# ChrisDud0257/SSL

Measured on AMD Instinct MI355X. Metric: SSG-loss edge-pixels/sec (fwd+bwd) 3x256x256 k_s=25 k_w=9, higher is better.
Workload: dtype f32; 1 GPU; C2: batch 16 x 3x256x256 per GPU, Laplacian mask, k_s=25 k_w=9 sigma=1.0, L1+KL w=1e3, SSGs materialised; launch=per-kernel, ranks_seen=1, edge_px_rank0=76466, images_rank0=16, input_checksum=c1391ff6908574f6, gradient_accumulation=fixed-point integer atomics (bit-reproducible, the shipped default), prewarm_steps=1949, parallelism=images sharded x1, no data-path collective

## Files before the change

include/ssg_hip.h:

```cpp
#ifndef SSG_HIP_H
#define SSG_HIP_H

#include <stddef.h>
#include <stdint.h>

#ifdef __cplusplus
extern "C" {
#endif

typedef void *ssg_stream_t;

#define SSG_E_BADARG (-1)
#define SSG_E_TOOLARGE (-2)
#define SSG_E_WORKSPACE (-3)
#define SSG_E_IMAGESMALL (-4)
#define SSG_E_ALIGN (-5)
#define SSG_E_PLAN (-6)

int ssg_abi_version(void);
const char *ssg_status_string(int status);
int ssg_device_status(ssg_stream_t stream);

int ssg_set_operator_plan_threshold(int positions);
int ssg_operator_pool_trim(void);
int ssg_compute_similarity(const float *image, const int *pos, float *out,
                           int mc, int psize, int ksize, int height, int width,
                           int channel, ssg_stream_t stream);

int ssg_compute_similarity_backward(const float *image, const float *grads,
                                    const int *pos, float *image_grads, int mc,
                                    int psize, int ksize, int height, int width,
                                    int channel, ssg_stream_t stream);

size_t ssg_edge_scratch_bytes(int B, int H, int W);
size_t ssg_forward_plan_bytes(int B, int H, int W, int capacity);
int ssg_set_dense_threshold(int edge_pixels_per_tile);
int ssg_set_overlap(int mode);
int ssg_last_overlap_assignment(void);
int ssg_set_tiny_step(int on);
int ssg_edge_list(const void *mask, int mask_kind, int mask_channels, int B,
                  int H, int W, int mask_stride, float lap_threshold,
                  int plan_ks ,
                  int *edges, int capacity, int *counts,
                  int *rank_map , int *tile_order ,
                  int *fwd_plan , void *scratch,
                  ssg_stream_t stream);

int ssg_edge_mask_laplacian(const float *gt, int B, int H, int W,
                            float lap_threshold, int mask_stride,
                            uint8_t *mask_out, ssg_stream_t stream);

int ssg_map_forward(const float *img, const float *img2, int B, int C, int H,
                    int W, const int *edges, const int *tile_order ,
                    const int *rank_map ,
                    const int *fwd_plan ,
                    const int *n_edges_dev, int n_rows,
                    int ks, int kw, float sigma, float eps, int generalization,
                    float *ssg, float *ssg2,
                    double *row_scale ,
                    ssg_stream_t stream);

size_t ssg_backward_scratch_bytes(int n_rows, int ks);
int ssg_map_backward(const float *img, int B, int C, int H, int W,
                     const int *edges, const int *tile_order ,
                     const int *rank_map ,
                     const int *fwd_plan ,
                     const int *n_edges_dev, int n_rows,
                     int ks, int kw, float sigma, int generalization,
                     const float *ssg, const float *grad_ssg, float *grad_img,
                     void *scratch , void *grad_fix ,
                     ssg_stream_t stream);

size_t ssg_grad_fix_bytes(int B, int C, int H, int W);

size_t ssg_loss_scratch_bytes(int B, int H, int W, int n_rows, int ks);
int ssg_loss_backward(const float *sr, int B, int C, int H, int W,
                      const int *edges, const int *tile_order ,
                      const int *rank_map ,
                      const int *fwd_plan ,
                      const int *n_edges_dev, int n_rows,
                      int ks, int kw, float sigma, int generalization,
                      float *ssg_sr, float *ssg_gt, float w_l1,
                      float w_kl, const float *upstream ,
                      float *loss_out, float *grad_sr ,
                      void *scratch, void *grad_fix ,
                      const double *row_scale , int rows_are_scratch, ssg_stream_t stream);

size_t ssg_criteria_scratch_bytes(void);
int ssg_criteria_sums(const float *pred, const float *target, size_t n, void *scratch, float *sums_out,
                      ssg_stream_t stream);
int ssg_criteria_grad(const float *pred, const float *target, size_t n, const float *coef, float *grad_pred,
                      ssg_stream_t stream);

size_t ssg_loss_workspace_bytes(int B, int H, int W, int capacity, int ks);
size_t ssg_loss_rows_bytes(int capacity, int ks);
size_t ssg_loss_tm_bytes(int capacity, int ks);
int ssg_loss_workspace_layout(int B, int H, int W, int capacity, int ks, int fused, size_t out[9]);
int ssg_loss_fwd_bwd(const float *sr, const float *gt, const void *mask,
                     int mask_kind, int mask_channels, int B, int C, int H,
                     int W, int ks, int kw, float sigma, float eps,
                     int generalization, float w_l1, float w_kl, int mask_stride,
                     float lap_threshold, int capacity, float *ssg_sr ,
                     float *ssg_gt, int *counts, float *loss_out, float *grad_sr,
                     void *workspace, size_t workspace_bytes,
                     void *grad_fix , ssg_stream_t stream);

int ssg_loss_step(const float *sr, const float *gt, const void *mask,
                  int mask_kind, int mask_channels, int B, int C, int H,
                  int W, int ks, int kw, float sigma, float eps,
                  int generalization, float w_l1, float w_kl, int mask_stride,
                  float lap_threshold, int capacity, float *ssg_sr ,
                  float *ssg_gt, int *counts, float *loss_out, float *grad_sr,
                  void *workspace, size_t workspace_bytes,
                  void *grad_fix , ssg_stream_t stream);

int ssg_augment_crop(const void *src, void *dst, int elem_bytes, int B, int C, int Hs, int Ws, int Ho, int Wo,
                     const int *params, ssg_stream_t stream);
int ssg_pool_swap(void *queue, void *batch, size_t sample_bytes, const int *slots, int b, ssg_stream_t stream);

int ssg_filter2d(const float *img, const float *kernels, float *out, int B, int C, int H, int W, int k, int n_kernels,
                 ssg_stream_t stream);
int ssg_diffjpeg(const float *img, float *out, int B, int H, int W, const float *quality_dev, float quality,
                 ssg_stream_t stream);
size_t ssg_usm_scratch_bytes(int B, int C, int H, int W);
int ssg_usm_sharp(const float *img, float *out, int B, int C, int H, int W, int radius, float sigma, float weight,
                  float threshold, void *scratch, size_t scratch_bytes, ssg_stream_t stream);

int ssg_resize(const float *img, float *out, int B, int C, int Hi, int Wi, int Ho, int Wo, int mode,
               double scale_factor_h, double scale_factor_w, ssg_stream_t stream);
int ssg_clamp_round(const float *img, float *out, size_t n, int clip, int rounds, ssg_stream_t stream);
int ssg_gaussian_noise(const float *img, float *out, const float *field_color, const float *field_gray,
                       const float *sigma, const float *gray, int B, int C, int H, int W, int clip, int rounds,
                       ssg_stream_t stream);
size_t ssg_poisson_scratch_bytes(int B);
int ssg_poisson_rates(const float *img, float *rate_color, float *rate_gray, float *vals, void *scratch, int B, int C,
                      int H, int W, ssg_stream_t stream);
int ssg_poisson_noise(const float *img, float *out, const float *draw_color, const float *draw_gray, const float *vals,
                      const float *scale, const float *gray, int B, int C, int H, int W, int clip, int rounds,
                      ssg_stream_t stream);

size_t ssg_ldl_workspace_bytes(int B, int H, int W);
int ssg_artifact_map(const float *output, const float *gt, const float *ema , int B, int C, int H, int W,
                     int k, float *w_out, void *workspace, size_t workspace_bytes, ssg_stream_t stream);
int ssg_artifact_map_backward(const float *output, const float *gt, const float *ema ,
                              const float *grad_w, int B, int C, int H, int W, int k, float *grad_output,
                              void *workspace, size_t workspace_bytes, ssg_stream_t stream);
int ssg_ldl_loss(const float *output, const float *gt, const float *ema , int B, int C, int H, int W,
                 int k, float loss_weight, int mean, float *loss_out, float *grad_output ,
                 void *workspace, size_t workspace_bytes, ssg_stream_t stream);
int ssg_local_variance(const float *residual, int B, int H, int W, int k, float *v_out ,
                       const float *grad_v , float *grad_residual , void *workspace,
                       size_t workspace_bytes, ssg_stream_t stream);

size_t ssg_bbl_workspace_bytes(int B, int C, int H, int W, int k, int stride);
int ssg_bbl_search(const float *x, const float *gt, int B, int C, int H, int W, int k, int stride, float alpha,
                   float beta, int *ind_out, float *p1_out , float *sel_out ,
                   void *workspace, size_t workspace_bytes, ssg_stream_t stream);
int ssg_bbl_loss(const float *x, const float *gt, int B, int C, int H, int W, int k, int stride, float alpha,
                 float beta, float loss_weight, int mean, float *loss_out, float *grad_x ,
                 int *ind_out , void *workspace, size_t workspace_bytes, ssg_stream_t stream);
int ssg_flat_mask(const float *img, int B, int H, int W, int k, float thresh, float *mask_out, ssg_stream_t stream);

#ifdef SSG_PROFILE
int ssg_set_profile_mask(int mask);
int ssg_prof_occupancy(int which);
int ssg_prof_strip_times(unsigned long long *host, int n);
int ssg_prof_set_lds_poison(int on, unsigned pattern);
#endif

const char *ssg_kernel_name(int ks, int kw, int backward);

#ifdef __cplusplus
}
#endif
#endif
```

ssl_amd/_lib.py:

```python
import ctypes
import os
import subprocess

_HERE = os.path.dirname(os.path.abspath(__file__))
CSRC = os.path.join(_HERE, "csrc")
SO_PATH = os.path.join(CSRC, "libssg_hip.so")
PROF_SO_PATH = os.path.join(CSRC, "libssg_hip_prof.so")
HEADER = os.path.join(os.path.dirname(_HERE), "include", "ssg_hip.h")

_vp, _i, _f, _sz = ctypes.c_void_p, ctypes.c_int, ctypes.c_float, ctypes.c_size_t

PROTOTYPES = {
    "ssg_abi_version": (_i, []),
    "ssg_status_string": (ctypes.c_char_p, [_i]),
    "ssg_compute_similarity": (_i, [_vp, _vp, _vp, _i, _i, _i, _i, _i, _i, _vp]),
    "ssg_compute_similarity_backward": (_i, [_vp, _vp, _vp, _vp, _i, _i, _i, _i, _i, _i, _vp]),
    "ssg_edge_scratch_bytes": (_sz, [_i, _i, _i]),
    "ssg_forward_plan_bytes": (_sz, [_i, _i, _i, _i]),
    "ssg_set_dense_threshold": (_i, [_i]),
    "ssg_set_overlap": (_i, [_i]),
    "ssg_last_overlap_assignment": (_i, []),
    "ssg_set_tiny_step": (_i, [_i]),
    "ssg_edge_list": (_i, [_vp, _i, _i, _i, _i, _i, _i, _f, _i, _vp, _i, _vp, _vp, _vp, _vp, _vp, _vp]),
    "ssg_edge_mask_laplacian": (_i, [_vp, _i, _i, _i, _f, _i, _vp, _vp]),
    "ssg_map_forward": (_i, [_vp, _vp, _i, _i, _i, _i, _vp, _vp, _vp, _vp, _vp, _i, _i, _i, _f, _f, _i, _vp, _vp,
                             _vp, _vp]),
    "ssg_backward_scratch_bytes": (_sz, [_i, _i]),
    "ssg_map_backward": (_i, [_vp, _i, _i, _i, _i, _vp, _vp, _vp, _vp, _vp, _i, _i, _i, _f, _i, _vp, _vp, _vp, _vp,
                              _vp, _vp]),
    "ssg_grad_fix_bytes": (_sz, [_i, _i, _i, _i]),
    "ssg_loss_scratch_bytes": (_sz, [_i, _i, _i, _i, _i]),
    "ssg_loss_backward": (_i, [_vp, _i, _i, _i, _i, _vp, _vp, _vp, _vp, _vp, _i, _i, _i, _f, _i, _vp, _vp, _f, _f,
                               _vp, _vp, _vp, _vp, _vp, _vp, _i, _vp]),
    "ssg_loss_workspace_bytes": (_sz, [_i, _i, _i, _i, _i]),
    "ssg_loss_rows_bytes": (_sz, [_i, _i]),
    "ssg_loss_tm_bytes": (_sz, [_i, _i]),
    "ssg_loss_workspace_layout": (_i, [_i, _i, _i, _i, _i, _i, ctypes.POINTER(ctypes.c_size_t)]),
    "ssg_filter2d": (_i, [_vp, _vp, _vp, _i, _i, _i, _i, _i, _i, _vp]),
    "ssg_diffjpeg": (_i, [_vp, _vp, _i, _i, _i, _vp, _f, _vp]),
    "ssg_usm_scratch_bytes": (_sz, [_i, _i, _i, _i]),
    "ssg_usm_sharp": (_i, [_vp, _vp, _i, _i, _i, _i, _i, _f, _f, _f, _vp, _sz, _vp]),
    "ssg_loss_fwd_bwd": (_i, [_vp, _vp, _vp, _i, _i, _i, _i, _i, _i, _i, _i, _f, _f, _i, _f, _f, _i, _f, _i, _vp, _vp,
                              _vp, _vp, _vp, _vp, _sz, _vp, _vp]),
    "ssg_loss_step": (_i, [_vp, _vp, _vp, _i, _i, _i, _i, _i, _i, _i, _i, _f, _f, _i, _f, _f, _i, _f, _i, _vp, _vp,
                           _vp, _vp, _vp, _vp, _sz, _vp, _vp]),
    "ssg_augment_crop": (_i, [_vp, _vp, _i, _i, _i, _i, _i, _i, _i, _vp, _vp]),
    "ssg_pool_swap": (_i, [_vp, _vp, _sz, _vp, _i, _vp]),
    "ssg_resize": (_i, [_vp, _vp, _i, _i, _i, _i, _i, _i, _i, ctypes.c_double, ctypes.c_double, _vp]),
    "ssg_clamp_round": (_i, [_vp, _vp, _sz, _i, _i, _vp]),
    "ssg_gaussian_noise": (_i, [_vp, _vp, _vp, _vp, _vp, _vp, _i, _i, _i, _i, _i, _i, _vp]),
    "ssg_poisson_scratch_bytes": (_sz, [_i]),
    "ssg_poisson_rates": (_i, [_vp, _vp, _vp, _vp, _vp, _i, _i, _i, _i, _vp]),
    "ssg_poisson_noise": (_i, [_vp, _vp, _vp, _vp, _vp, _vp, _vp, _i, _i, _i, _i, _i, _i, _vp]),
    "ssg_kernel_name": (ctypes.c_char_p, [_i, _i, _i]),
    "ssg_ldl_workspace_bytes": (_sz, [_i, _i, _i]),
    "ssg_artifact_map": (_i, [_vp, _vp, _vp, _i, _i, _i, _i, _i, _vp, _vp, _sz, _vp]),
    "ssg_artifact_map_backward": (_i, [_vp, _vp, _vp, _vp, _i, _i, _i, _i, _i, _vp, _vp, _sz, _vp]),
    "ssg_ldl_loss": (_i, [_vp, _vp, _vp, _i, _i, _i, _i, _i, _f, _i, _vp, _vp, _vp, _sz, _vp]),
    "ssg_local_variance": (_i, [_vp, _i, _i, _i, _i, _vp, _vp, _vp, _vp, _sz, _vp]),
    "ssg_bbl_workspace_bytes": (_sz, [_i, _i, _i, _i, _i, _i]),
    "ssg_bbl_search": (_i, [_vp, _vp, _i, _i, _i, _i, _i, _i, _f, _f, _vp, _vp, _vp, _vp, _sz, _vp]),
    "ssg_bbl_loss": (_i, [_vp, _vp, _i, _i, _i, _i, _i, _i, _f, _f, _f, _i, _vp, _vp, _vp, _vp, _sz, _vp]),
    "ssg_flat_mask": (_i, [_vp, _i, _i, _i, _i, _f, _vp, _vp]),
    "ssg_ref_compute_similarity": (None, [_vp, _vp, _vp, _i, _i, _i, _i, _i, _i]),
    "ssg_ref_compute_similarity_backward": (None, [_vp, _vp, _vp, _vp, _i, _i, _i, _i, _i, _i]),
    "ssg_last_status": (_i, []),
    "ssg_device_status": (_i, [_vp]),
    "ssg_set_operator_plan_threshold": (_i, [_i]),
    "ssg_operator_pool_trim": (_i, []),
    "ssg_criteria_scratch_bytes": (_sz, []),
    "ssg_criteria_sums": (_i, [_vp, _vp, _sz, _vp, _vp, _vp]),
    "ssg_criteria_grad": (_i, [_vp, _vp, _sz, _vp, _vp, _vp]),
}
PROF_PROTOTYPES = {"ssg_set_profile_mask": (_i, [_i]), "ssg_prof_occupancy": (_i, [_i]),
                   "ssg_prof_set_lds_poison": (_i, [_i, ctypes.c_uint])}
CXX_SYMBOLS = ("_Z19_compute_similarityPKfPKiPfiiiiii", "_Z28_compute_similarity_backwardPKfS0_PKiPfiiiiii")


def build(force=False, verbose=False):
    cmd = ["make", "-C", CSRC, "-j4"] + (["-B"] if force else [])
    out = subprocess.run(cmd, stdout=subprocess.PIPE, stderr=subprocess.STDOUT, text=True)
    if verbose or out.returncode:
        print(out.stdout)
    if out.returncode:
        raise RuntimeError("building libssg_hip.so failed (see output above)")
    return SO_PATH


_lib = None
_prof = None


def _load(path, prototypes):
    import torch
    if torch.cuda.is_available():
        torch.cuda.init()
    if not os.path.exists(path):
        raise RuntimeError(
            f"{path} is missing: run `python -c 'import __graft_entry__ as g; g.build()'` "
            "(or `make -C ssl_amd/csrc`).  ssl_amd has no CPU / PyTorch fallback for the SSG kernels.")
    L = ctypes.CDLL(path)
    for name, (res, args) in prototypes.items():
        fn = getattr(L, name)
        fn.restype = res
        fn.argtypes = args
    for name in CXX_SYMBOLS:
        getattr(L, name)
    return L


def lib():
    global _lib
    if _lib is None:
        _lib = _load(SO_PATH, PROTOTYPES)
    return _lib


def lib_prof():
    global _prof
    if _prof is None:
        _prof = _load(PROF_SO_PATH, dict(PROTOTYPES, **PROF_PROTOTYPES))
    return _prof


class profile_build:

    def __enter__(self):
        global _lib
        self._saved = _lib
        _lib = lib_prof()
        return _lib

    def __exit__(self, *exc):
        global _lib
        _lib.ssg_set_profile_mask(0)
        _lib = self._saved
        return False


def check(status):
    if status != 0:
        raise RuntimeError(f"libssg_hip: {lib().ssg_status_string(status).decode()} (status {status})")
```

ssl_amd/csrc/ssg_api.hip:

```cpp
#include "../../include/ssg_hip.h"

#include <atomic>
#include <cstdlib>
#include <mutex>

#include "ssg_common.hpp"

namespace ssg {
int launch_fwd(const FwdParams &p, hipStream_t st);
int launch_bwd(const BwdParams &p, hipStream_t st);
unsigned bwd_grid(const BwdParams &p);
size_t bwd_max_partials(int B, int H, int W, int n_rows);
int launch_loss_finalize(const LossFinalize &f, hipStream_t st);
const char *fwd_kernel_name(int ks, int kw);
const char *bwd_kernel_name(int ks, int kw);
size_t edge_scratch_bytes(int B, int H, int W);
int launch_edge_list(const void *mask, int kind, int mask_channels, int B, int H, int W, int stride, float thr,
                     int *edges, int capacity, int *counts, int *rank, int *order, int *plan, int dense_thr,
                     int plan_tile_rows, void *scratch, void *zero_a, size_t zero_a_bytes, void *zero_b,
                     size_t zero_b_bytes, void *zero_c, size_t zero_c_bytes, hipStream_t st);
size_t fwd_plan_bytes(int B, int H, int W, int capacity);
int fwd_plan_order_offset(int B, int H, int W);
struct DenseParams {
  const float *img[2];
// ... 70 lines not shown
    if (v < 0) v = 0;
    g_dense_thr.store(v, std::memory_order_relaxed);
  }
  return v;
}

static std::atomic<int> g_tiny_step{1};
extern "C" int ssg_set_tiny_step(int on) { return g_tiny_step.exchange(on != 0 ? 1 : 0, std::memory_order_relaxed); }
extern "C" int ssg_set_operator_plan_threshold(int positions);
extern "C" int ssg_set_dense_threshold(int edge_pixels_per_tile) {
  const int prev = dense_threshold();
  g_dense_thr.store(edge_pixels_per_tile > 0 ? edge_pixels_per_tile : 0, std::memory_order_relaxed);
  return prev;
}

#ifdef SSG_PROFILE
static std::atomic<int> g_dbg{-1};
static int dbg_mask() {
  int v = g_dbg.load(std::memory_order_relaxed);
  if (v < 0) {
    v = env_int("SSG_DEBUG_SKIP", 0);
    if (v < 0) v = 0;
    g_dbg.store(v, std::memory_order_relaxed);
  }
  return v;
}
namespace ssg { int strip_occupancy(); int strip_times(unsigned long long *host, int n); }
static std::atomic<int> g_lds_poison_on{0};
static std::atomic<unsigned> g_lds_poison_pat{0};
__global__ __launch_bounds__(256) void lds_poison_kernel(unsigned pat, int words) {
  extern __shared__ unsigned s_poison[];
  volatile unsigned *w = s_poison;
  for (int i = threadIdx.x; i < words; i += 256) w[i] = pat;
}
namespace ssg {
void prof_poison_lds(hipStream_t st) {
  if (!g_lds_poison_on.load(std::memory_order_relaxed)) return;
  constexpr int BYTES = 160 * 1024;
  static std::atomic<unsigned long long> lds_set{0};
  if (ensure_dynamic_lds(lds_poison_kernel, BYTES, lds_set)) return;
  lds_poison_kernel<<<dim3(1024), dim3(256), BYTES, st>>>(g_lds_poison_pat.load(std::memory_order_relaxed), BYTES / 4);
}
}
extern "C" int ssg_prof_set_lds_poison(int on, unsigned pattern) {
  const int prev = g_lds_poison_on.load(std::memory_order_relaxed);
  g_lds_poison_pat.store(pattern, std::memory_order_relaxed);
  g_lds_poison_on.store(on ? 1 : 0, std::memory_order_relaxed);
  return prev;
}
extern "C" int ssg_prof_strip_times(unsigned long long *host, int n) { return ssg::strip_times(host, n); }
extern "C" int ssg_prof_occupancy(int which) { return which == 0 ? ssg::strip_occupancy() : -1; }
extern "C" int ssg_set_profile_mask(int mask) {
  const int prev = dbg_mask();
  g_dbg.store(mask > 0 ? mask : 0, std::memory_order_relaxed);
  return prev;
}
#else
static constexpr int dbg_mask() { return 0; }
#endif

struct SideStream {
  hipStream_t side = nullptr;
  hipEvent_t forked = nullptr, joined = nullptr, gate = nullptr, gate2 = nullptr;
};
static std::atomic<int> g_overlap{-1};
static int overlap_mode() {
  int v = g_overlap.load(std::memory_order_relaxed);
  if (v < 0) {
    v = env_int("SSG_OVERLAP", 3);
    v = v < 0 ? 0 : (v > 3 ? 3 : v);
    g_overlap.store(v, std::memory_order_relaxed);
  }
  return v;
}

static bool stream_capturing(hipStream_t st) {
  hipStreamCaptureStatus cs = hipStreamCaptureStatusNone;
  return hipStreamIsCapturing(st, &cs) == hipSuccess && cs != hipStreamCaptureStatusNone;
}

struct PlanHint {
  int *host = nullptr, *dev = nullptr;
};
static PlanHint plan_hint(bool allocate_never = false) {
  constexpr int MAXDEV = 64;
  static std::mutex mu;
  static PlanHint tab[MAXDEV];
  int dev = 0;
  if (hipGetDevice(&dev) != hipSuccess || dev < 0 || dev >= MAXDEV) return PlanHint{};
  std::lock_guard<std::mutex> lk(mu);
  if (!tab[dev].host) {
    if (allocate_never) return PlanHint{};
    void *h = nullptr, *d = nullptr;
    if (hipHostMalloc(&h, 64, hipHostMallocMapped) != hipSuccess) return PlanHint{};
    ((int *)h)[0] = ((int *)h)[1] = -1;
    if (hipHostGetDevicePointer(&d, h, 0) != hipSuccess) {
      (void)hipHostFree(h);
      return PlanHint{};
    }
    tab[dev] = PlanHint{(int *)h, (int *)d};
  }
  return tab[dev];
}
namespace ssg {
int *plan_hint_device_word(hipStream_t st) {
  if (overlap_mode() != 3) return nullptr;
  return plan_hint(stream_capturing(st)).dev;
}
}

struct Schedule {
  hipStream_t st = nullptr;
  bool may_fork = false;
  int assign = 0;
  bool chains = false;
  bool gated = false;
  int rows_hint = 0;
  SideStream *side = nullptr;
  bool open = false;
  hipStream_t dense() const { return open && assign == 2 ? side->side : st; }
  hipStream_t direct() const { return open && assign == 1 ? side->side : st; }
};

static Schedule schedule(hipStream_t st, int ks, bool chains) {
  Schedule s;
  s.st = st;
  const int mode = overlap_mode();
  int n_sparse = -1, n_tiles = -1;
  if (mode == 3) {
    const PlanHint h = plan_hint(true);
    if (h.host) {
      n_sparse = ((volatile int *)h.host)[0];
      n_tiles = ((volatile int *)h.host)[1];
    }
  }
  const bool known = n_sparse >= 0 && n_tiles >= 0;
  const bool direct_longer = known && (long long)n_sparse * 38 > (long long)n_tiles * 740;
  s.assign = mode == 3 ? (direct_longer ? 2 : 1) : mode;
  s.rows_hint = n_sparse > 0 ? n_sparse : 0;
  s.may_fork = ks <= 25 && mode != 0;
  const bool free = mode == 3 && known && (direct_longer || n_tiles <= 512);
  s.chains = chains && s.may_fork && (free || !stream_capturing(st));
  s.gated = !free && s.assign == 1;
  return s;
}

static thread_local int t_last_assignment = 0;
extern "C" int ssg_last_overlap_assignment(void) { return t_last_assignment; }
extern "C" int ssg_set_overlap(int mode) {
  const int prev = overlap_mode();
  g_overlap.store(mode < 0 ? 0 : (mode > 3 ? 3 : mode), std::memory_order_relaxed);
  return prev;
}
static SideStream *side_stream() {
  constexpr int MAXDEV = 64;
  thread_local SideStream tab[MAXDEV];
  int dev = 0;
  if (hipGetDevice(&dev) != hipSuccess || dev < 0 || dev >= MAXDEV) return nullptr;
  SideStream &s = tab[dev];
  if (!s.side) {
    if (hipStreamCreateWithFlags(&s.side, hipStreamNonBlocking) != hipSuccess ||
        hipEventCreateWithFlags(&s.forked, hipEventDisableTiming) != hipSuccess ||
        hipEventCreateWithFlags(&s.joined, hipEventDisableTiming) != hipSuccess ||
        hipEventCreateWithFlags(&s.gate, hipEventDisableTiming) != hipSuccess ||
        hipEventCreateWithFlags(&s.gate2, hipEventDisableTiming) != hipSuccess) {
      s.side = nullptr;
      return nullptr;
    }
  }
  return &s;
}
static void fork_side(Schedule &s, bool skip = false) {
  s.side = s.may_fork && !skip ? side_stream() : nullptr;
  s.open = s.side && hipEventRecord(s.side->forked, s.st) == hipSuccess &&
           hipStreamWaitEvent(s.side->side, s.side->forked, 0) == hipSuccess;
  t_last_assignment = s.open ? s.assign : 0;
}
static int join_side(Schedule &s) {
  if (!s.open) return 0;
  s.open = false;
  int rc = (int)hipEventRecord(s.side->joined, s.side->side);
  if (!rc) rc = (int)hipStreamWaitEvent(s.st, s.side->joined, 0);
  return rc;
}

static int *device_status_word() {
  constexpr int MAXDEV = 64;
  static std::mutex mu;
  static int *tab[MAXDEV] = {};
  int dev = 0;
  if (hipGetDevice(&dev) != hipSuccess || dev < 0 || dev >= MAXDEV) return nullptr;
  std::lock_guard<std::mutex> lk(mu);
  if (!tab[dev]) {
    int *w = nullptr;
    if (hipMalloc(&w, sizeof(int)) != hipSuccess) return nullptr;
    if (hipMemset(w, 0, sizeof(int)) != hipSuccess) {
      (void)hipFree(w);
      return nullptr;
    }
    tab[dev] = w;
  }
  return tab[dev];
}

static bool sizes_ok(int ks, int kw) { return ks > 0 && kw > 0 && (ks & 1) && (kw & 1) && kw <= ks; }

static size_t align_up(size_t v, size_t a) { return (v + a - 1) / a * a; }

static int bwd_qsplit() {
  static int v = -1;
  if (v < 0) {
    v = env_int("SSG_BWD_QSPLIT", 0);
    if (v < 0) v = 0;
    if (v > 25) v = 25;
  }
  return v;
}

static size_t split_scratch_bytes(int n_rows, int ks) {
  const size_t n = (size_t)(n_rows > 0 ? n_rows : 1);
  return align_up(sizeof(float) * n * ks * ks, 256) + 3 * align_up(sizeof(float) * n, 256);
}

struct TileMajor {
  float *rows[2] = {nullptr, nullptr};
  int slots = 0;
};
static bool strips_enabled() {
  static int v = -1;
  if (v < 0) {
    v = env_int("SSG_STRIPS", 1) != 0;
  }
  return v != 0;
}
static bool tile_major_enabled() {
  static int v = -1;
  if (v < 0) {
    v = env_int("SSG_TILE_MAJOR", 1) != 0;
  }
  return v != 0;
}

static int split_tm_tiles(const BwdParams &p, const TileMajor *tm) {
  if (!tm || tm->slots <= 0) return 0;
  const int mt = dense_max_tiles(p.B, p.H, p.W, p.ks);
  return tm->slots < mt ? tm->slots : mt;
}

static bool split_row_classes(const BwdParams &p, int n_tm) {
  return p.mode == GRAD_LOSS && n_tm == 0 && p.row_scale && p.ks <= 25;
}

static int split_backward(BwdParams p, const int *rank, const int *plan, void *scratch, Schedule &sc,
                          const LossFinalize *fin = nullptr, bool *fin_done = nullptr, const TileMajor *tm = nullptr) {
  const hipStream_t st = sc.st;
  float *G = (float *)scratch;
  const size_t nfl = align_up(sizeof(float) * (size_t)(p.n_host > 0 ? p.n_host : 1), 256);
  float *sum_b = (float *)((char *)scratch + align_up(sizeof(float) * (size_t)p.n_host * p.ks * p.ks, 256));
  float *gmax_part = (float *)((char *)sum_b + nfl);
  float *dot = (float *)((char *)gmax_part + nfl);
  const int n_tm = split_tm_tiles(p, tm);
  GrowParams g{};
  g.mode = p.mode;
  g.gin = p.gin;
  g.ssg = p.ssg;
  g.ssg2 = p.ssg2;
  g.row_scale = p.row_scale;
  g.rows_scratch = p.rows_scratch;
  g.n_dev = p.n_dev;
  g.n_host = p.n_host;
  g.C = p.C;
  g.sigma = p.sigma;
  g.generalization = p.generalization;
  g.w_l1 = p.w_l1;
  g.w_kl = p.w_kl;
  g.upstream = p.upstream;
  g.G = p.grad ? G : nullptr;
  g.sum_b = p.grad ? sum_b : nullptr;
  g.partials = p.partials;
  g.gmax_part = p.gfix ? gmax_part : nullptr;
  if (n_tm > 0) {
    g.grid_cap = 4096;
    g.tm_hdr = plan + 1;
    g.tm_slots = tm->slots;
    g.sparse_order = plan + fwd_plan_order_offset(p.B, p.H, p.W);
  }
  const size_t n_fix = (size_t)p.B * p.C * p.H * p.W;
  const bool apriori = p.gfix && p.mode == GRAD_LOSS && n_tm == 0;
  const bool classes = split_row_classes(p, n_tm);
  if (sc.chains && !sc.open && classes && p.grad) fork_side(sc, dbg_mask() & ((1 << 27) | (1 << 28) | (1 << 29)));
  const bool gated = sc.open && sc.gated;
  if (apriori) {
    g.gmax_part = nullptr;
    g.fix_word = (unsigned *)(p.gfix + n_fix);
  }
  int rc = gated ? (int)hipEventRecord(sc.side->gate, st) : 0;
  if (!rc && !(dbg_mask() & (1 << 29))) {
    if (classes) {
      GrowParams gd = g;
      gd.only = 1;
      rc = launch_grad_rows(gd, p.ks, p.kw, sc.dense());
      GrowParams gs = g;
      gs.only = 2;
      gs.grid_cap = 4096;
      gs.tm_hdr = plan + 1;
      gs.tm_slots = 0;
      gs.sparse_order = plan + fwd_plan_order_offset(p.B, p.H, p.W);
      gs.partials = p.partials + 2 * (size_t)grow_grid(p.n_host);
      if (!rc) rc = launch_grad_rows(gs, p.ks, p.kw, sc.direct());
    } else {
      rc = launch_grad_rows(g, p.ks, p.kw, st);
    }
  }
  if (!rc && n_tm > 0) {
    TmRowsParams t{};
    t.tm[0] = tm->rows[0];
    t.tm[1] = tm->rows[1];
    t.row_scale = p.row_scale;
    t.rank = rank;
    t.n_dense = plan + 1;
    t.tiles = plan + 4;
    t.n_tiles = n_tm;
    t.tm_slots = tm->slots;
    t.n_dev = p.n_dev;
    t.n_host = p.n_host;
    t.B = p.B;
    t.H = p.H;
    t.W = p.W;
    t.C = p.C;
    t.sigma = p.sigma;
    t.w_l1 = p.w_l1;
    t.w_kl = p.w_kl;
    t.upstream = p.upstream;
    t.dot = dot;
    t.sum_b = sum_b;
    t.partials = p.partials + 2 * (size_t)grow_grid(p.n_host);
    t.gmax_part = p.gfix ? gmax_part + grow_grid(p.n_host) : nullptr;
    if (!p.rows_scratch) {
      t.out[0] = p.ssg;
      t.out[1] = p.ssg2;
    }
    rc = (dbg_mask() & (1 << 29)) ? 0 : launch_rows_tm(t, p.ks, p.kw, st);
  }
  if (rc || !p.grad) return rc;
  if (p.gfix && !apriori) {
    rc = launch_grad_fix_reduce(gmax_part, (int)grow_grid(p.n_host) + rows_tm_parts(n_tm), p.gfix, n_fix, st);
    if (rc) return rc;
  }
  const float *grows = p.mode == GRAD_D ? p.gin : G;
  DenseBwdParams d{};
  d.img = p.img;
  d.grad = p.grad;
  d.gfix = p.gfix;
  d.G = grows;
  d.sum_b = sum_b;
  d.rank = rank;
  d.n_dense = plan + 1;
  d.tiles = plan + 4;
  d.max_tiles = dense_max_tiles(p.B, p.H, p.W, p.ks);
  d.n_dev = p.n_dev;
  d.n_host = p.n_host;
  d.B = p.B;
  d.H = p.H;
  d.W = p.W;
  d.qsplit = bwd_qsplit();
  d.dbg = p.dbg;
  d.status = device_status_word();
  if (n_tm > 0) {
    d.tm[0] = tm->rows[0];
    d.tm[1] = tm->rows[1];
    d.row_scale = p.row_scale;
    d.dot = dot;
    d.tm_slots = tm->slots;
    d.sigma = p.sigma;
    d.w_l1 = p.w_l1;
    d.w_kl = p.w_kl;
    d.upstream = p.upstream;
  }
  if (gated) {
    rc = (int)hipStreamWaitEvent(sc.direct(), sc.side->gate, 0);
    if (!rc) rc = (int)hipEventRecord(sc.side->gate2, sc.dense());
  }
  if (!sc.open) {
    fork_side(sc, dbg_mask() & ((1 << 27) | (1 << 28)));
    if (!rc && fin && sc.open) {
      rc = launch_loss_finalize(*fin, sc.side->side);
      if (!rc) *fin_done = true;
    }
  }
  if (!rc && !(dbg_mask() & (1 << 27))) rc = launch_bwd_dense(d, p.ks, p.kw, p.C, sc.dense());
  if (!rc && !(dbg_mask() & (1 << 28))) {
    BwdParams s = p;
    s.mode = GRAD_D;
    s.gin = grows;
    s.order = plan + fwd_plan_order_offset(p.B, p.H, p.W);
    s.n_dev = plan;
    s.partials = nullptr;
    s.rows_hint = sc.rows_hint;
    rc = launch_bwd(s, sc.direct());
  }
  if (!rc && gated && fin) {
    rc = (int)hipStreamWaitEvent(sc.direct(), sc.side->gate2, 0);
    if (!rc) rc = launch_loss_finalize(*fin, sc.direct());
    if (!rc) *fin_done = true;
  }
  const int rcj = join_side(sc);
  return rc ? rc : rcj;
}

static int det_begin(BwdParams &p, void *grad_fix, hipStream_t st, bool prezeroed = false) {
  p.gfix = nullptr;
  if (!grad_fix || !p.grad) return 0;
  p.gfix = (long long *)grad_fix;
  if (prezeroed) return 0;
  return (int)hipMemsetAsync(grad_fix, 0, sizeof(long long) * ((size_t)p.B * p.C * p.H * p.W + 8), st);
}
static int det_end(const BwdParams &p, hipStream_t st, bool assign = false, const LossFinalize *fin = nullptr, bool *fin_done = nullptr) {
  if (!p.gfix) return 0;
  const int rc = launch_grad_fix_flush(p.gfix, p.grad, (size_t)p.B * p.C * p.H * p.W, assign ? 1 : 0, st, fin);
  if (!rc && fin && fin_done) *fin_done = true;
  return rc;
}

constexpr int OP_PLAN_FROM_DEFAULT = 8192;
static std::atomic<int> g_op_plan_from{-1};
static int op_plan_from() {
  int v = g_op_plan_from.load(std::memory_order_relaxed);
  if (v < 0) {
    v = env_int("SSG_OP_PLAN_FROM", OP_PLAN_FROM_DEFAULT);
    if (v <= 0) v = 0x7fffffff;
    g_op_plan_from.store(v, std::memory_order_relaxed);
  }
  return v;
}

static hipMemPool_t op_pool() {
  constexpr int MAXDEV = 64;
  static std::mutex mu;
  static hipMemPool_t tab[MAXDEV] = {};
  static bool failed[MAXDEV] = {};
  int dev = 0;
  if (hipGetDevice(&dev) != hipSuccess || dev < 0 || dev >= MAXDEV) return nullptr;
  std::lock_guard<std::mutex> lk(mu);
  if (!tab[dev] && !failed[dev]) {
    hipMemPoolProps props{};
    props.allocType = hipMemAllocationTypePinned;
    props.location.type = hipMemLocationTypeDevice;
    props.location.id = dev;
    hipMemPool_t pool = nullptr;
    if (hipMemPoolCreate(&pool, &props) != hipSuccess) {
      failed[dev] = true;
      (void)hipGetLastError();
      return nullptr;
    }
    unsigned long long keep = ~0ull;
    (void)hipMemPoolSetAttribute(pool, hipMemPoolAttrReleaseThreshold, &keep);
    tab[dev] = pool;
// ... 711 lines not shown
```

ssl_amd/csrc/ssg_grow.hip:

```cpp
#include "ssg_common.hpp"

namespace ssg {

template <int KS, int KW>
__global__ __launch_bounds__(256) void ssg_grad_rows(GrowParams p) {
  constexpr int P = KS * KS, HP = KS / 2, HK = KW / 2, EPL = (P + 63) / 64;
  __shared__ float sred[12];
  const int lane = threadIdx.x & 63, wv = threadIdx.x >> 6;
  const int nrows = rows_to_do(p.n_dev, p.n_host);
  if (p.fix_word && blockIdx.x == 0 && threadIdx.x == 0) {
    *p.fix_word = __float_as_uint(loss_grad_bound(p.sigma, p.C, KW, p.w_l1, p.w_kl, p.upstream, nrows, P));
  }
  const bool via_list = p.tm_hdr && p.sparse_order && (p.only == 2 || tm_active(p.tm_hdr, p.tm_slots, nrows));
  const int n_list = via_list ? (p.tm_hdr[-1] < nrows ? p.tm_hdr[-1] : nrows) : 0;
  const int live_rows = (nrows + 3) / 4 < p.ngroups ? (nrows + 3) / 4 : p.ngroups;
  const int live_groups = via_list ? (n_list + 3) / 4 : live_rows;
  for (int g = live_groups + blockIdx.x * 256 + threadIdx.x; g < p.ngroups; g += gridDim.x * 256) {
    if (p.gmax_part) p.gmax_part[g] = 0.f;
    if (p.mode == GRAD_LOSS) {
      p.partials[2 * g] = 0.f;
      p.partials[2 * g + 1] = 0.f;
    }
  }
  for (int grp = blockIdx.x; grp < live_groups; grp += gridDim.x) {
  const int k4 = grp * 4 + wv;
  const int n = via_list ? (k4 < n_list ? (p.sparse_order[k4] & ORDER_MASK) : nrows) : k4;
  float l1p = 0.f, klp = 0.f, gmax = 0.f;
  const bool tm_row = n < nrows && p.row_scale && p.mode == GRAD_LOSS && p.row_scale[n] < 0.0;
  const bool other_chain = p.only == 1 && n < nrows && p.row_scale[n] == 0.0;
  if (n < nrows && !tm_row && !other_chain) {
    const size_t base = (size_t)n * P;
    float va[EPL], vg[EPL];
    const float *src_a = p.mode == GRAD_D ? p.gin : p.ssg;
#pragma unroll
    for (int k = 0; k < EPL; ++k) {
      const int e = lane + 64 * k;
      va[k] = e < P ? src_a[base + e] : 0.f;
    }
    if (p.mode != GRAD_D) {
      const float *src_b = p.mode == GRAD_S ? p.gin : p.ssg2;
#pragma unroll
      for (int k = 0; k < EPL; ++k) {
        const int e = lane + 64 * k;
        vg[k] = e < P ? src_b[base + e] : 0.f;
      }
      if (p.row_scale && p.mode == GRAD_LOSS) {
        const double sa = p.row_scale[n], sb2 = p.row_scale[(size_t)p.n_host + n];
        if (sa != 0.0) {
#pragma unroll
          for (int k = 0; k < EPL; ++k) {
            const int e = lane + 64 * k;
            va[k] = (float)(sa * (double)va[k]);
            if (e < P && !p.rows_scratch) const_cast<float *>(p.ssg)[base + e] = va[k];
          }
        }
        if (sb2 != 0.0) {
#pragma unroll
          for (int k = 0; k < EPL; ++k) {
            const int e = lane + 64 * k;
            vg[k] = (float)(sb2 * (double)vg[k]);
            if (e < P && !p.rows_scratch) const_cast<float *>(p.ssg2)[base + e] = vg[k];
          }
        }
      }
      const float invM = 1.f / ((float)nrows * (float)P);
      const float u1 = p.upstream ? p.upstream[0] : 1.f, u2 = p.upstream ? p.upstream[1] : 1.f;
      const float w1m = p.w_l1 * invM * u1, w2m = p.w_kl * invM * u2;
      float dot = 0.f;
#pragma unroll
      for (int k = 0; k < EPL; ++k) {
        const int e = lane + 64 * k;
        float g = 0.f;
        if (e < P) g = p.mode == GRAD_S ? vg[k] : criteria_elem(va[k], vg[k], w1m, w2m, l1p, klp);
        vg[k] = g;
        dot = __builtin_fmaf(g, va[k], dot);
      }
      dot = p.generalization ? wave_sum(dot) : 0.f;
      const float kfac = 1.f / (p.sigma * (float)(p.C * KW * KW));
#pragma unroll
      for (int k = 0; k < EPL; ++k) va[k] = -(va[k] * kfac) * (vg[k] - dot);
    }
    float sb = 0.f, gm = 0.f;
#pragma unroll
    for (int k = 0; k < EPL; ++k) {
      const int e = lane + 64 * k;
      if (e < P) {
        const int py = e / KS, px = e - py * KS;
        if (e == HP * KS + HP) va[k] = 0.f;
        gm = fmaxf(gm, fabsf(va[k]));
        const bool border = py < HK || py > KS - 1 - HK || px < HK || px > KS - 1 - HK;
        if (border) sb += va[k];
        if (p.G && p.mode != GRAD_D) p.G[base + e] = va[k];
      }
    }
    if (p.sum_b) {
      sb = wave_sum(sb);
      if (lane == 0) p.sum_b[n] = sb;
    }
    gmax = gm;
  }
  if (p.gmax_part) {
#pragma unroll
    for (int o = 32; o > 0; o >>= 1) gmax = fmaxf(gmax, __shfl_xor(gmax, o, 64));
    if (lane == 0) sred[8 + wv] = gmax;
    __syncthreads();
    if (threadIdx.x == 0) p.gmax_part[grp] = fmaxf(fmaxf(sred[8], sred[9]), fmaxf(sred[10], sred[11]));
  }
  if (p.mode == GRAD_LOSS) {
    l1p = wave_sum(l1p);
    klp = wave_sum(klp);
    if (lane == 0) {
      sred[wv] = l1p;
      sred[4 + wv] = klp;
    }
    __syncthreads();
    if (threadIdx.x == 0) {
      p.partials[2 * grp] = (sred[0] + sred[1]) + (sred[2] + sred[3]);
      p.partials[2 * grp + 1] = (sred[4] + sred[5]) + (sred[6] + sred[7]);
    }
  }
  if (gridDim.x < (unsigned)live_groups) __syncthreads();
  }
}

template <int KS, int KW>
__global__ __launch_bounds__(1024) void ssg_rows_tm(TmRowsParams p) {
  constexpr int P = KS * KS, HP = KS / 2, HK = KW / 2, NQ = 8, TY = 4, TX = 32, UNR = 7;
  static_assert(KS % UNR == 0 && TY * TX == TM_PX, "offset rows in groups of 7; 4 x 32 tiles");
  __shared__ float red[8][NQ][TM_PX];
  __shared__ double redk[NQ][TM_PX];
  __shared__ float wred[3][16];
  const int lane = threadIdx.x & 63, wv = threadIdx.x >> 6, ck = wv & 1, part = wv >> 1;
  const int tslot = blockIdx.x;
  if (tslot >= dense_tile_count(p.n_dense) || p.n_dense[1] != TY ||
      !tm_active(p.n_dense, p.tm_slots, rows_to_do(p.n_dev, p.n_host))) {
    if (threadIdx.x < 2) {
      p.partials[2 * (2 * tslot + threadIdx.x)] = 0.f;
      p.partials[2 * (2 * tslot + threadIdx.x) + 1] = 0.f;
      if (p.gmax_part) p.gmax_part[2 * tslot + threadIdx.x] = 0.f;
    }
    return;
  }
  const int H = p.H, W = p.W;
  const int tx_n = (W + TX - 1) / TX, ty_n = (H + TY - 1) / TY;
  const int tile = dense_tile_id(dense_tile_at(p.n_dense, p.tiles, p.B * ty_n * tx_n, tslot));
  const int b = tile / (tx_n * ty_n), tr = tile - b * tx_n * ty_n;
  const int ty0 = (tr / tx_n) * TY, tx0 = (tr % tx_n) * TX;
  const int nrows = rows_to_do(p.n_dev, p.n_host);
  const int y = ty0 + tm_pixel_row(ck, lane), x = tx0 + tm_pixel_col(lane);
  int r = (y < H && x < W) ? p.rank[((size_t)b * H + y) * W + x] : -1;
  if (r >= nrows) r = -1;
  const TmScale sa = tm_scale(r >= 0 ? p.row_scale[r] : 0.0), sb = tm_scale(r >= 0 ? p.row_scale[(size_t)p.n_host + r] : 0.0);
  const float invM = 1.f / ((float)nrows * (float)P);
  const float u1 = p.upstream ? p.upstream[0] : 1.f, u2 = p.upstream ? p.upstream[1] : 1.f;
  const float w1m = p.w_l1 * invM * u1, w2m = p.w_kl * invM * u2;
  const float cl = 1e-10f;
  const float *pa = p.tm[0] + (size_t)tslot * P * TM_PX + ck * 64 + lane;
  const float *pb = p.tm[1] + (size_t)tslot * P * TM_PX + ck * 64 + lane;
  float l1 = 0.f, d1 = 0.f, d2 = 0.f, bs = 0.f, bg = 0.f, m1 = 0.f, m2 = 0.f;
  double kld = 0.0;
  const int qy0 = (KS * part) / NQ, qy1 = (KS * (part + 1)) / NQ;
  for (int qy = qy0; qy < qy1; ++qy) {
    const bool yb = qy < HK || qy > KS - 1 - HK, yc = qy == HP;
    float kl = 0.f;
#pragma unroll 1
    for (int g0 = 0; g0 < KS; g0 += UNR) {
      float ea[UNR], eb[UNR];
#pragma unroll
      for (int j = 0; j < UNR; ++j) {
        ea[j] = __builtin_nontemporal_load(pa + (size_t)(qy * KS + g0 + j) * TM_PX);
        eb[j] = __builtin_nontemporal_load(pb + (size_t)(qy * KS + g0 + j) * TM_PX);
      }
#pragma unroll
      for (int j = 0; j < UNR; ++j) {
        const int qx = g0 + j;
        const float a = tm_apply(ea[j], sa), t = tm_apply(eb[j], sb);
        const float ac = fmaxf(a, cl), bc = fmaxf(t, cl);
        l1 += fabsf(a - t);
        const float rc = __builtin_amdgcn_rcpf(ac);
        const float r0 = bc * rc;
        const float ratio = __builtin_fmaf(__builtin_fmaf(-r0, ac, bc), rc, r0);
        kl += bc * (0.69314718056f * __builtin_amdgcn_logf(ratio));
        const float sg = __builtin_amdgcn_fmed3f((a - t) * 0x1p126f, -1.f, 1.f);
        const float bz = a >= cl ? bc : 0.f;
        d1 = __builtin_fmaf(sg, a, d1);
        d2 += bz;
        const float gs = __builtin_fmaf(w1m * sg, a, -w2m * bz);
        const float bm = (yb || qx < HK || qx > KS - 1 - HK) ? 1.f : 0.f, cm = (qx == HP && yc) ? 0.f : 1.f;
        bs = __builtin_fmaf(a, bm, bs);
        bg = __builtin_fmaf(gs, bm, bg);
        m1 = fmaxf(m1, a * cm);
        m2 = fmaxf(m2, fabsf(a - bz) * cm);
      }
    }
    kld += (double)kl;
  }
  red[0][part][ck * 64 + lane] = l1;
  redk[part][ck * 64 + lane] = kld;
  red[2][part][ck * 64 + lane] = d1;
  red[3][part][ck * 64 + lane] = d2;
  red[4][part][ck * 64 + lane] = bs;
  red[5][part][ck * 64 + lane] = bg;
  red[6][part][ck * 64 + lane] = m1;
  red[7][part][ck * 64 + lane] = m2;
  __syncthreads();
  float l1w = 0.f, klw = 0.f, gb = 0.f;
  if (part == 0) {
    const int px = ck * 64 + lane;
    float v[8];
#pragma unroll
    for (int k = 0; k < 6; ++k) {
      if (k == 1) continue;
      float t = red[k][0][px];
#pragma unroll
      for (int j = 1; j < NQ; ++j) t += red[k][j][px];
      v[k] = t;
    }
    {
      double t = redk[0][px];
#pragma unroll
      for (int j = 1; j < NQ; ++j) t += redk[j][px];
      v[1] = (float)t;
    }
#pragma unroll
    for (int k = 6; k < 8; ++k) {
      float t = red[k][0][px];
#pragma unroll
      for (int j = 1; j < NQ; ++j) t = fmaxf(t, red[k][j][px]);
      v[k] = t;
    }
    const float kfac = 1.f / (p.sigma * (float)(p.C * KW * KW));
    v[2] *= w1m;
    v[3] *= -w2m;
    const float dot = v[2] + v[3];
    if (r >= 0) {
      p.dot[r] = dot;
      p.sum_b[r] = -kfac * (v[5] - dot * v[4]);
    }
    gb = kfac * (v[6] * (fabsf(w1m) + fabsf(v[2]) + fabsf(v[3] + w2m)) + fabsf(w2m) * v[7]) * 1.0001f;
    l1w = wave_sum(v[0]);
    klw = wave_sum(v[1]);
#pragma unroll
    for (int o = 32; o > 0; o >>= 1) gb = fmaxf(gb, __shfl_xor(gb, o, 64));
    if (lane == 0) {
      wred[0][ck] = l1w;
      wred[1][ck] = klw;
      wred[2][ck] = gb;
    }
  }
  __syncthreads();
  if (threadIdx.x < 2) {
    p.partials[2 * (2 * tslot + threadIdx.x)] = wred[0][threadIdx.x];
    p.partials[2 * (2 * tslot + threadIdx.x) + 1] = wred[1][threadIdx.x];
    if (p.gmax_part) p.gmax_part[2 * tslot + threadIdx.x] = wred[2][threadIdx.x];
  }
}

template <int KS, int KW>
__global__ __attribute__((amdgpu_flat_work_group_size(512, 512), amdgpu_waves_per_eu(4, 4))) void ssg_rows_tm_mat(TmRowsParams p) {
  constexpr int P = KS * KS, HP = KS / 2, HK = KW / 2, NQ = 8, TY = 4, TX = 32, QMAX = (KS + NQ - 1) / NQ;
  constexpr int CPX = 64, NR = 2, RING = 128, PITCH = RING + 4, SEG = 16, NIT = (KS + NR - 1) / NR;
  static_assert(TY * TX == TM_PX && QMAX == 7, "4 x 32 tiles; at most 7 offsets of a row per part");
  static_assert(NR * KS + SEG - 1 <= RING, "a hand-over's new offsets + the carried ones fit the ring");
  typedef float f4 __attribute__((ext_vector_type(4)));
  extern __shared__ __attribute__((aligned(16))) float lds[];
  float *stage = lds;
  int *prow = (int *)(stage + 2 * CPX * PITCH);
  float *red = lds;
  double *redk = (double *)(red + 8 * NQ * CPX);
  float *wred = (float *)(redk + NQ * CPX);
  const int lane = threadIdx.x & 63, part = threadIdx.x >> 6;
  const int slot = blockIdx.x;
  const int tslot = slot >> 1, ck = slot & 1;
  if (tslot >= dense_tile_count(p.n_dense) || p.n_dense[1] != TY ||
      !tm_active(p.n_dense, p.tm_slots, rows_to_do(p.n_dev, p.n_host))) {
// ... 339 lines not shown
```

Before: 64.81 million edge-px/s.

## Software-pipeline grad-rows kernel with buffer-load prefetch of next row group

Restructures ssg_grad_rows so that for KS=25 each wave prefetches the next row's SSG data with raw buffer loads (bounded by a buffer resource, so dead rows read zero) while computing the current row, and fetches row indices and scales two iterations ahead through scalar uniform loads. Row index and scale lookups are split into helpers and made wave-uniform via readfirstlane. It also adds an API knob to force the row-pass grid size and an optional compile-time per-CU grid cap for the gated chain, which is off by default. The aim is to hide global-load latency in the row pass, at the cost of extra registers for the double buffers, which may lower occupancy.

```diff
diff --git a/include/ssg_hip.h b/include/ssg_hip.h
--- a/include/ssg_hip.h
+++ b/include/ssg_hip.h
@@ -37,6 +37,7 @@
 int ssg_set_dense_threshold(int edge_pixels_per_tile);
 int ssg_set_overlap(int mode);
 int ssg_last_overlap_assignment(void);
+int ssg_set_row_pass_grid(int workgroups);
 int ssg_set_tiny_step(int on);
 int ssg_edge_list(const void *mask, int mask_kind, int mask_channels, int B,
                   int H, int W, int mask_stride, float lap_threshold,
diff --git a/ssl_amd/_lib.py b/ssl_amd/_lib.py
--- a/ssl_amd/_lib.py
+++ b/ssl_amd/_lib.py
@@ -20,6 +20,7 @@
     "ssg_set_dense_threshold": (_i, [_i]),
     "ssg_set_overlap": (_i, [_i]),
     "ssg_last_overlap_assignment": (_i, []),
+    "ssg_set_row_pass_grid": (_i, [_i]),
     "ssg_set_tiny_step": (_i, [_i]),
     "ssg_edge_list": (_i, [_vp, _i, _i, _i, _i, _i, _i, _f, _i, _vp, _i, _vp, _vp, _vp, _vp, _vp, _vp]),
     "ssg_edge_mask_laplacian": (_i, [_vp, _i, _i, _i, _f, _i, _vp, _vp]),
diff --git a/ssl_amd/csrc/ssg_api.hip b/ssl_amd/csrc/ssg_api.hip
--- a/ssl_amd/csrc/ssg_api.hip
+++ b/ssl_amd/csrc/ssg_api.hip
@@ -246,6 +246,27 @@
   g_overlap.store(mode < 0 ? 0 : (mode > 3 ? 3 : mode), std::memory_order_relaxed);
   return prev;
 }
+#ifndef SSG_ROW_PASS_WGS_PER_CU
+#define SSG_ROW_PASS_WGS_PER_CU 0
+#endif
+constexpr int ROW_PASS_WGS_PER_CU = SSG_ROW_PASS_WGS_PER_CU;
+static int device_cu_count() {
+  constexpr int MAXDEV = 64;
+  static std::atomic<int> tab[MAXDEV];
+  int dev = 0;
+  if (hipGetDevice(&dev) != hipSuccess || dev < 0 || dev >= MAXDEV) return 0;
+  int v = tab[dev].load(std::memory_order_relaxed);
+  if (v <= 0) {
+    if (hipDeviceGetAttribute(&v, hipDeviceAttributeMultiprocessorCount, dev) != hipSuccess || v <= 0) return 0;
+    tab[dev].store(v, std::memory_order_relaxed);
+  }
+  return v;
+}
+static std::atomic<int> g_row_pass_grid{0};
+extern "C" int ssg_set_row_pass_grid(int workgroups) {
+  return g_row_pass_grid.exchange(workgroups > 0 ? workgroups : 0, std::memory_order_relaxed);
+}
+
 static SideStream *side_stream() {
   constexpr int MAXDEV = 64;
   thread_local SideStream tab[MAXDEV];
@@ -389,14 +410,17 @@
     g.fix_word = (unsigned *)(p.gfix + n_fix);
   }
   int rc = gated ? (int)hipEventRecord(sc.side->gate, st) : 0;
+  const int forced_grid = g_row_pass_grid.load(std::memory_order_relaxed);
+  if (forced_grid > 0) g.grid_cap = forced_grid;
   if (!rc && !(dbg_mask() & (1 << 29))) {
     if (classes) {
       GrowParams gd = g;
       gd.only = 1;
+      if (gated && forced_grid <= 0 && ROW_PASS_WGS_PER_CU > 0) gd.grid_cap = ROW_PASS_WGS_PER_CU * device_cu_count();
       rc = launch_grad_rows(gd, p.ks, p.kw, sc.dense());
       GrowParams gs = g;
       gs.only = 2;
-      gs.grid_cap = 4096;
+      gs.grid_cap = forced_grid > 0 ? forced_grid : 4096;
       gs.tm_hdr = plan + 1;
       gs.tm_slots = 0;
       gs.sparse_order = plan + fwd_plan_order_offset(p.B, p.H, p.W);
diff --git a/ssl_amd/csrc/ssg_grow.hip b/ssl_amd/csrc/ssg_grow.hip
--- a/ssl_amd/csrc/ssg_grow.hip
+++ b/ssl_amd/csrc/ssg_grow.hip
@@ -2,50 +2,105 @@
 
 namespace ssg {
 
-template <int KS, int KW>
-__global__ __launch_bounds__(256) void ssg_grad_rows(GrowParams p) {
-  constexpr int P = KS * KS, HP = KS / 2, HK = KW / 2, EPL = (P + 63) / 64;
-  __shared__ float sred[12];
-  const int lane = threadIdx.x & 63, wv = threadIdx.x >> 6;
-  const int nrows = rows_to_do(p.n_dev, p.n_host);
-  if (p.fix_word && blockIdx.x == 0 && threadIdx.x == 0) {
-    *p.fix_word = __float_as_uint(loss_grad_bound(p.sigma, p.C, KW, p.w_l1, p.w_kl, p.upstream, nrows, P));
-  }
-  const bool via_list = p.tm_hdr && p.sparse_order && (p.only == 2 || tm_active(p.tm_hdr, p.tm_slots, nrows));
-  const int n_list = via_list ? (p.tm_hdr[-1] < nrows ? p.tm_hdr[-1] : nrows) : 0;
-  const int live_rows = (nrows + 3) / 4 < p.ngroups ? (nrows + 3) / 4 : p.ngroups;
-  const int live_groups = via_list ? (n_list + 3) / 4 : live_rows;
-  for (int g = live_groups + blockIdx.x * 256 + threadIdx.x; g < p.ngroups; g += gridDim.x * 256) {
-    if (p.gmax_part) p.gmax_part[g] = 0.f;
-    if (p.mode == GRAD_LOSS) {
-      p.partials[2 * g] = 0.f;
-      p.partials[2 * g + 1] = 0.f;
-    }
-  }
-  for (int grp = blockIdx.x; grp < live_groups; grp += gridDim.x) {
+template <class T>
+__device__ __forceinline__ T uniform_load(const T *ptr, int idx) {
+  const unsigned long long a = (unsigned long long)ptr;
+  const unsigned lo = __builtin_amdgcn_readfirstlane((int)(unsigned)a), hi = __builtin_amdgcn_readfirstlane((int)(unsigned)(a >> 32));
+  return ((const __attribute__((address_space(4))) T *)(((unsigned long long)hi << 32) | lo))[__builtin_amdgcn_readfirstlane(idx)];
+}
+
+struct GrowRowIdx {
+  int n;
+  double sa, sb2;
+  bool live;
+};
+
+__device__ __forceinline__ int grow_row_word(const GrowParams &p, int grp, int live_groups, int wv, bool via_list,
+                                             int n_list) {
   const int k4 = grp * 4 + wv;
-  const int n = via_list ? (k4 < n_list ? (p.sparse_order[k4] & ORDER_MASK) : nrows) : k4;
-  float l1p = 0.f, klp = 0.f, gmax = 0.f;
-  const bool tm_row = n < nrows && p.row_scale && p.mode == GRAD_LOSS && p.row_scale[n] < 0.0;
-  const bool other_chain = p.only == 1 && n < nrows && p.row_scale[n] == 0.0;
-  if (n < nrows && !tm_row && !other_chain) {
-    const size_t base = (size_t)n * P;
-    float va[EPL], vg[EPL];
-    const float *src_a = p.mode == GRAD_D ? p.gin : p.ssg;
+  return via_list ? uniform_load(p.sparse_order, grp < live_groups && k4 < n_list ? k4 : 0) : 0;
+}
+__device__ __forceinline__ int grow_row_n(int word, int grp, int live_groups, int wv, int nrows, bool via_list, int n_list) {
+  const int k4 = grp * 4 + wv;
+  if (grp >= live_groups) return nrows;
+  if (!via_list) return k4;
+  return k4 < n_list ? (word & ORDER_MASK) : nrows;
+}
+
+__device__ __forceinline__ void grow_row_scales(const GrowParams &p, int n, int nrows, double &sa, double &sb2) {
+  sa = sb2 = 0.0;
+  if ((p.row_scale && p.mode == GRAD_LOSS) || p.only == 1) {
+    sa = uniform_load(p.row_scale, n < nrows ? n : 0);
+    sb2 = uniform_load(p.row_scale + (size_t)p.n_host, n < nrows ? n : 0);
+  }
+}
+__device__ __forceinline__ GrowRowIdx grow_row_idx(const GrowParams &p, int n, int nrows, double sa, double sb2) {
+  GrowRowIdx r;
+  r.n = n;
+  r.sa = n < nrows ? sa : 0.0;
+  r.sb2 = n < nrows ? sb2 : 0.0;
+  const bool tm_row = p.row_scale && p.mode == GRAD_LOSS && r.sa < 0.0;
+  const bool other_chain = p.only == 1 && r.sa == 0.0;
+  r.live = n < nrows && !tm_row && !other_chain;
+  return r;
+}
+
+template <int KS>
+__device__ __forceinline__ void grow_row_load(const GrowParams &p, const GrowRowIdx &r, int lane,
+                                              float (&va)[(KS * KS + 63) / 64], float (&vg)[(KS * KS + 63) / 64]) {
+  constexpr int P = KS * KS, EPL = (P + 63) / 64;
+#pragma unroll
+  for (int k = 0; k < EPL; ++k) va[k] = vg[k] = 0.f;
+  if (!r.live) return;
+  const size_t base = (size_t)r.n * P;
+  const float *src_a = p.mode == GRAD_D ? p.gin : p.ssg;
+#pragma unroll
+  for (int k = 0; k < EPL; ++k) {
+    const int e = lane + 64 * k;
+    va[k] = e < P ? src_a[base + e] : 0.f;
+  }
+  if (p.mode != GRAD_D) {
+    const float *src_b = p.mode == GRAD_S ? p.gin : p.ssg2;
 #pragma unroll
     for (int k = 0; k < EPL; ++k) {
       const int e = lane + 64 * k;
-      va[k] = e < P ? src_a[base + e] : 0.f;
-    }
+      vg[k] = e < P ? src_b[base + e] : 0.f;
+    }
+  }
+}
+
+constexpr int BUF_RSRC_WORD3 = 0x00020000;
+template <int KS>
+__device__ __forceinline__ void grow_row_prefetch(const GrowParams &p, const GrowRowIdx &r, int lane,
+                                                  float (&va)[(KS * KS + 63) / 64], float (&vg)[(KS * KS + 63) / 64]) {
+  constexpr int P = KS * KS, EPL = (P + 63) / 64;
+  const int live = __builtin_amdgcn_readfirstlane(r.live ? 1 : 0);
+  const size_t base = (size_t)__builtin_amdgcn_readfirstlane(live ? r.n : 0) * P;
+  const float *src_a = p.mode == GRAD_D ? p.gin : p.ssg;
+  const float *src_b = p.mode == GRAD_D ? p.gin : (p.mode == GRAD_S ? p.gin : p.ssg2);
+  const int bytes_a = live ? P * 4 : 0, bytes_b = live && p.mode != GRAD_D ? P * 4 : 0;
+  const __amdgpu_buffer_rsrc_t ra = __builtin_amdgcn_make_buffer_rsrc((void *)(src_a + base), 0, bytes_a, BUF_RSRC_WORD3);
+  const __amdgpu_buffer_rsrc_t rb = __builtin_amdgcn_make_buffer_rsrc((void *)(src_b + base), 0, bytes_b, BUF_RSRC_WORD3);
+#pragma unroll
+  for (int k = 0; k < EPL; ++k)
+    va[k] = __builtin_bit_cast(float, __builtin_amdgcn_raw_buffer_load_b32(ra, (lane + 64 * k) * 4, 0, 0));
+#pragma unroll
+  for (int k = 0; k < EPL; ++k)
+    vg[k] = __builtin_bit_cast(float, __builtin_amdgcn_raw_buffer_load_b32(rb, (lane + 64 * k) * 4, 0, 0));
+}
+
+template <int KS, int KW>
+__device__ __forceinline__ void grow_group(const GrowParams &p, int grp, const GrowRowIdx &r, float (&va)[(KS * KS + 63) / 64],
+                                           float (&vg)[(KS * KS + 63) / 64], int nrows, int lane, int wv, float *sred,
+                                           bool sred_reused) {
+  constexpr int P = KS * KS, HP = KS / 2, HK = KW / 2, EPL = (P + 63) / 64;
+  const int n = r.n;
+  float l1p = 0.f, klp = 0.f, gmax = 0.f;
+  if (r.live) {
+    const size_t base = (size_t)n * P;
     if (p.mode != GRAD_D) {
-      const float *src_b = p.mode == GRAD_S ? p.gin : p.ssg2;
-#pragma unroll
-      for (int k = 0; k < EPL; ++k) {
-        const int e = lane + 64 * k;
-        vg[k] = e < P ? src_b[base + e] : 0.f;
-      }
       if (p.row_scale && p.mode == GRAD_LOSS) {
-        const double sa = p.row_scale[n], sb2 = p.row_scale[(size_t)p.n_host + n];
+        const double sa = r.sa, sb2 = r.sb2;
         if (sa != 0.0) {
 #pragma unroll
           for (int k = 0; k < EPL; ++k) {
@@ -119,8 +174,82 @@
       p.partials[2 * grp + 1] = (sred[4] + sred[5]) + (sred[6] + sred[7]);
     }
   }
-  if (gridDim.x < (unsigned)live_groups) __syncthreads();
-  }
+  if (sred_reused) __syncthreads();
+}
+
+template <int KS, int KW>
+__global__ __launch_bounds__(256) void ssg_grad_rows(GrowParams p) {
+  constexpr int P = KS * KS, EPL = (P + 63) / 64;
+  constexpr bool PIPE = KS == 25;
+  __shared__ float sred[12];
+  const int lane = threadIdx.x & 63, wv = __builtin_amdgcn_readfirstlane((int)(threadIdx.x >> 6));
+  const int nrows = __builtin_amdgcn_readfirstlane(rows_to_do(p.n_dev, p.n_host));
+  if (p.fix_word && blockIdx.x == 0 && threadIdx.x == 0) {
+    *p.fix_word = __float_as_uint(loss_grad_bound(p.sigma, p.C, KW, p.w_l1, p.w_kl, p.upstream, nrows, P));
+  }
+  const bool via_list = __builtin_amdgcn_readfirstlane(
+      p.tm_hdr && p.sparse_order && (p.only == 2 || tm_active(p.tm_hdr, p.tm_slots, nrows)) ? 1 : 0) != 0;
+  const int n_list = __builtin_amdgcn_readfirstlane(via_list ? (p.tm_hdr[-1] < nrows ? p.tm_hdr[-1] : nrows) : 0);
+  const int live_rows = (nrows + 3) / 4 < p.ngroups ? (nrows + 3) / 4 : p.ngroups;
+  const int live_groups = via_list ? (n_list + 3) / 4 : live_rows;
+  for (int g = live_groups + blockIdx.x * 256 + threadIdx.x; g < p.ngroups; g += gridDim.x * 256) {
+    if (p.gmax_part) p.gmax_part[g] = 0.f;
+    if (p.mode == GRAD_LOSS) {
+      p.partials[2 * g] = 0.f;
+      p.partials[2 * g + 1] = 0.f;
+    }
+  }
+  const int stride = __builtin_amdgcn_readfirstlane((int)gridDim.x);
+  const bool sred_reused = gridDim.x < (unsigned)live_groups;
+  float va[EPL], vg[EPL];
+  if (!PIPE) {
+    for (int grp = blockIdx.x; grp < live_groups; grp += stride) {
+      const int n = grow_row_n(grow_row_word(p, grp, live_groups, wv, via_list, n_list), grp, live_groups, wv, nrows,
+                               via_list, n_list);
+      double sa, sb2;
+      grow_row_scales(p, n, nrows, sa, sb2);
+      const GrowRowIdx r = grow_row_idx(p, n, nrows, sa, sb2);
+      grow_row_load<KS>(p, r, lane, va, vg);
+      grow_group<KS, KW>(p, grp, r, va, vg, nrows, lane, wv, sred, sred_reused);
+    }
+    return;
+  }
+#define GROW_ROW_N(g) grow_row_n(grow_row_word(p, (g), live_groups, wv, via_list, n_list), (g), live_groups, wv, nrows, via_list, n_list)
+  const int g0 = (int)blockIdx.x;
+  if (g0 >= live_groups) return;
+  GrowRowIdx r0, r1;
+  {
+    const int n0 = GROW_ROW_N(g0), n1 = GROW_ROW_N(g0 + stride);
+    double sa, sb2;
+    grow_row_scales(p, n0, nrows, sa, sb2);
+    r0 = grow_row_idx(p, n0, nrows, sa, sb2);
+    grow_row_scales(p, n1, nrows, sa, sb2);
+    r1 = grow_row_idx(p, n1, nrows, sa, sb2);
+  }
+  int n2 = GROW_ROW_N(g0 + 2 * stride);
+#undef GROW_ROW_N
+  float na[EPL], ng[EPL];
+  grow_row_prefetch<KS>(p, r0, lane, va, vg);
+#define GROW_TRIP(cur_a, cur_g, nxt_a, nxt_g)                                                             \
+  {                                                                                                       \
+    const int w3 = grow_row_word(p, grp + 3 * stride, live_groups, wv, via_list, n_list);                 \
+    double sa2, sb2;                                                                                      \
+    grow_row_scales(p, n2, nrows, sa2, sb2);                                                              \
+    grow_row_prefetch<KS>(p, r1, lane, nxt_a, nxt_g);                                                     \
+    grow_group<KS, KW>(p, grp, r0, cur_a, cur_g, nrows, lane, wv, sred, sred_reused);                     \
+    r0 = r1;                                                                                              \
+    r1 = grow_row_idx(p, n2, nrows, sa2, sb2);                                                            \
+    n2 = grow_row_n(w3, grp + 3 * stride, live_groups, wv, nrows, via_list, n_list);                      \
+  }
+  for (int grp = g0;;) {
+    GROW_TRIP(va, vg, na, ng)
+    grp += stride;
+    if (grp >= live_groups) break;
+    GROW_TRIP(na, ng, va, vg)
+    grp += stride;
+    if (grp >= live_groups) break;
+  }
+#undef GROW_TRIP
 }
 
 template <int KS, int KW>
```

Measured after the change: 65.13 million edge-px/s, median of 6. No clear change (+0.5%).
